# clayne/CPU-Raytracer

Measured on AMD Instinct MI355X. Metric: Mrays/s (primary+shadow+reflection+refraction), higher is better.
Workload: dtype f32

## Files before the change

### cpu-raytracer_amd/csrc/rtx_api.hip

```cpp
#include <hip/hip_runtime.h>
#include <stdio.h>
#include <stdlib.h>
#include <string.h>
#include <math.h>
#include <string>
#include <vector>
#include <algorithm>
#include <type_traits>

#include "../../include/rtx.h"
#include "rtx_device.h"
#include "rtx_math.h"
#include "rtx_libm.h"
#include "rtx_texture.h"
#include "rtx_trace.h"
#include "rtx_shade.h"
#include "rtx_packet.h"
#include "rtx_present.h"
#include "rtx_update.h"
#include "rtx_refit.h"
#include "rtx_build.h"
#include "rtx_normals.h"
#include "rtx_query.h"
#include "rtx_nearest.h"
// ... 153 lines not shown
    K.shade_grid = (int)knob_int("RTX_SHADE_GRID", 4, 1, 64);
    K.lane_from_level = (int)knob_int("RTX_LANE_FROM_LEVEL", -1, 0, 1 << 20);
    K.lane_from_level_any = (int)knob_int("RTX_LANE_FROM_LEVEL_ANY", -1, 0, 1 << 20);
    K.split_items = (int)knob_int("RTX_PK_SPLIT", 256, 0, 1 << 16);
    if (K.split_items > 0) K.split_items = (K.split_items + 63) & ~63;
    K.resolve_block = (int)knob_int("RTX_RESOLVE_BLOCK", 256, 64, 256);
    if (K.resolve_block != 64 && K.resolve_block != 128 && K.resolve_block != 256) K.resolve_block = 256;
    K.pk4_order = (int)knob_int("RTX_PK4_ORDER", 1, 0, 1);
    K.merge_any = knob_int("RTX_SERIAL_MERGE_ANY", 1, 0, 1) != 0;
    K.no_wide = knob_int("RTX_PK_WIDE", 1, 0, 1) == 0;
    K.lpt = (int)knob_int("RTX_PK_LPT", -1, -1, 1);
    K.graph = knob_int("RTX_GRAPH", 0, 0, 1) != 0;
    K.no_wide_closest = knob_int("RTX_PK_WIDE_CLOSEST", 1, 0, 1) == 0;
    K.fuse_shade = knob_int("RTX_FUSE_SHADE", 0, 0, 1) != 0;
    K.update_small_max = (int)knob_int("RTX_UPDATE_SMALL_MAX", RTX_UPDATE_SMALL_MAX, 0, RTX_UPDATE_SMALL_MAX);
    K.tex_pass_levels = (int)knob_int("RTX_TEX_PASS_LEVELS", rtxt::DEFAULT_PASS_LEVELS, 1, rtxt::MAX_PASS_LEVELS);
    c->nearest_fetch = knob_int("RTX_NEAREST_FETCH", 1, 0, 1) != 0;
    c->query_grid = (int)knob_int("RTX_QUERY_GRID", 0, 0, 1 << 20);
    K.fail_item_alloc = knob_int("RTX_DEBUG_FAIL_ITEM_ALLOC", 0, 0, 1) != 0;
    int bpc = 0;
    hipOccupancyMaxActiveBlocksPerMultiprocessor(&bpc, k_trace_fast<false>, RTX_TRACE_BLOCK, 0);
    c->trace_blocks_closest = c->n_cu * (bpc > 0 ? bpc : 2);
    hipOccupancyMaxActiveBlocksPerMultiprocessor(&bpc, k_trace_fast<true>, RTX_TRACE_BLOCK, 0);
    c->trace_blocks_any = c->n_cu * (bpc > 0 ? bpc : 2);
    hipOccupancyMaxActiveBlocksPerMultiprocessor(&bpc, k_trace<false, true>, RTX_TRACE_BLOCK, 0);
    c->trace_blocks_count = c->n_cu * (bpc > 0 ? bpc : 2);
    if (K.fuse_shade) hipOccupancyMaxActiveBlocksPerMultiprocessor(&bpc, k_packet<false, false, false, true, false>, RTX_PK_BLOCK, 0);
    else              hipOccupancyMaxActiveBlocksPerMultiprocessor(&bpc, k_packet<false, false>, RTX_PK_BLOCK, 0);
    c->pk_blocks_closest = (c->n_cu * (bpc > 0 ? bpc : 4) + 1) & ~1;
    hipOccupancyMaxActiveBlocksPerMultiprocessor(&bpc, k_packet<true, false>, RTX_PK_BLOCK, 0);
    c->pk_blocks_any = (c->n_cu * (bpc > 0 ? bpc : 4) + 1) & ~1;
    {
        const double f = knob_real("RTX_PK_GRID_SCALE", 1.0, 0.05, 16.0);
        if (f != 1.0) { c->pk_blocks_closest = ((int)(c->pk_blocks_closest * f) + 1) & ~1; c->pk_blocks_any = ((int)(c->pk_blocks_any * f) + 1) & ~1; }
        const double fa = knob_real("RTX_PK_GRID_ANY", 0.0, 0.05, 64.0), fc = knob_real("RTX_PK_GRID_CLOSEST", 0.0, 0.05, 64.0);
        if (fa > 0.0) c->pk_blocks_any = ((int)(c->n_cu * fa) + 1) & ~1;
        if (fc > 0.0) c->pk_blocks_closest = ((int)(c->n_cu * fc) + 1) & ~1;
    }
    {
        const int g = RTX_PK_CLASSES * RTX_WAVE / RTX_PK_BLOCK > 1 ? RTX_PK_CLASSES * RTX_WAVE / RTX_PK_BLOCK : 1;
        c->pk_blocks_any = (c->pk_blocks_any + g - 1) / g * g; c->pk_blocks_closest = (c->pk_blocks_closest + g - 1) / g * g;
        if (c->pk_blocks_any < g) c->pk_blocks_any = g;
        if (c->pk_blocks_closest < g) c->pk_blocks_closest = g;
    }
    long long max_threads = (long long)(c->trace_blocks_closest > c->trace_blocks_any ? c->trace_blocks_closest : c->trace_blocks_any) * RTX_TRACE_BLOCK;
    if ((long long)c->trace_blocks_count * RTX_TRACE_BLOCK > max_threads) max_threads = (long long)c->trace_blocks_count * RTX_TRACE_BLOCK;
    if ((long long)c->pk_blocks_any * RTX_PK_BLOCK > max_threads) max_threads = (long long)c->pk_blocks_any * RTX_PK_BLOCK;
    if ((long long)c->pk_blocks_closest * RTX_PK_BLOCK > max_threads) max_threads = (long long)c->pk_blocks_closest * RTX_PK_BLOCK;
    c->q.pk_defer_t0 = (int)knob_int("RTX_PK_DEFER", 8, 0, 64);
    c->q.pk_defer_leaf = (int)knob_int("RTX_PK_DEFER_LEAF", c->q.pk_defer_t0 / 2, 0, 64);
    c->q.pk_defer_t0_closest = (int)knob_int("RTX_PK_DEFER_CLOSEST", 64, 0, 64);
    c->q.pk_closest_asm = (int)knob_int("RTX_PK_CLOSEST_ASM", 1, 0, 1);
    c->q.pk_defer_t0_primary = (int)knob_int("RTX_PK_DEFER_PRIMARY", c->q.pk_closest_asm ? 4 : 64, 0, 64);
    c->q.pk_order = (int)knob_int("RTX_PK_ORDER", 1, 0, 1);
    c->q.prof_level = (int)knob_int("RTX_LANE_PROF_LEVEL", 2, 0, 100 + RTX_MAX_LEVELS);
    c->q.pk_defer_grow = (int)knob_int("RTX_PK_GROW", 3, 0, 31);
    c->q.spill_threads = (int)max_threads;
    rc = ensure(c, c->d_spill, (size_t)c->q.spill_threads * (RTX_MAX_STACK - RTX_LDS_STACK) * 4 * 3);
    if (!rc) rc = ensure(c, c->d_pk_fifo, (size_t)c->q.spill_threads * RTX_PK_FIFO * 8);
    { int ib = 0; hipOccupancyMaxActiveBlocksPerMultiprocessor(&ib, k_items, RTX_ITEM_BLOCK, 0); c->item_blocks = c->n_cu * (ib > 0 ? ib : 4);
      const double f = knob_real("RTX_ITEM_GRID", 0.0, 0.05, 64.0); if (f > 0.0) c->item_blocks = (int)(c->n_cu * f) > 0 ? (int)(c->n_cu * f) : 1; }
    c->q.pk_items = nullptr; c->q.pk_item_count = nullptr; c->q.pk_item_cap = 0;
    if (rc) { rtx_destroy(c); return rc; }
    *out_ctx = c;
    return RTX_OK;
}

extern "C" int rtx_destroy(rtx_ctx * c) {
    if (!c) return RTX_ERR_INVALID_ARG;
    hipSetDevice(c->cfg.device);
    if (c->stream) hipStreamSynchronize(c->stream);
    for (hipEvent_t e : c->event_pool) hipEventDestroy(e);
    if (c->graph_exec) { hipGraphExecDestroy(c->graph_exec); c->graph_exec = nullptr; }
    if (c->order_stream) { hipStreamSynchronize(c->order_stream); hipStreamDestroy(c->order_stream); hipEventDestroy(c->ev_cost); hipEventDestroy(c->ev_order); }
    if (c->any_stream) { hipStreamSynchronize(c->any_stream); hipStreamDestroy(c->any_stream); }
    if (c->ev_shade0) hipEventDestroy(c->ev_shade0);
    if (c->ev_shade_last) hipEventDestroy(c->ev_shade_last);
    if (c->ev_any_done) hipEventDestroy(c->ev_any_done);
    if (c->own_stream) hipStreamDestroy(c->own_stream);
    delete c;
    return RTX_OK;
}

static bool validate_tree(const rtx_bvh_node * nodes, int node_count, int64_t primitive_count, int * max_inner_depth = nullptr, int * max_leaf_count = nullptr) {
    if (node_count < 1) return false;
    std::vector<unsigned char> seen((size_t)node_count, 0);
    std::vector<std::pair<int, int>> stack(1, std::make_pair(0, 0));
    int deepest = -1, biggest = 0;
    while (!stack.empty()) {
        const int i = stack.back().first, d = stack.back().second; stack.pop_back();
        if (seen[i]) return false;
        seen[i] = 1;
        const int cnt = nodes[i].count & 0x3fffffff, f = nodes[i].left_or_first;
        if (cnt > 0) { if (f < 0 || (int64_t)f + cnt > primitive_count) return false; if (cnt > biggest) biggest = cnt; }
        else { if (f < 0 || f + 1 >= node_count) return false; if (d > deepest) deepest = d; stack.push_back(std::make_pair(f, d + 1)); stack.push_back(std::make_pair(f + 1, d + 1)); }
    }
    if (max_inner_depth) *max_inner_depth = deepest;
    if (max_leaf_count) *max_leaf_count = biggest;
    return true;
}


struct BlasStaged { DevBlas B; rtx_ctx::BlasHost H; };

template <typename T> static int stage_array(rtx_ctx * c, std::vector<DevBuf> & arrays, const void * src, size_t copy, size_t bytes, const T ** out) {
    DevBuf b;
// ... 2149 lines not shown
```

### cpu-raytracer_amd/csrc/rtx_packet.h

```cpp
#pragma once
#include "rtx_math.h"
#include "rtx_device.h"
#include "rtx_trace.h"
#include "rtx_shade.h"

#define RTX_PK_CLASSES  8
#ifndef RTX_PK_WAVES_ANY
#define RTX_PK_WAVES_ANY 5
#endif
#ifndef RTX_PK_WAVES_SPLIT
#define RTX_PK_WAVES_SPLIT 5
#endif
#ifndef RTX_PK_WAVES_CLOSEST
#define RTX_PK_WAVES_CLOSEST 4
#endif
#ifndef RTX_PK_CHUNK
#define RTX_PK_CHUNK 64u
#endif
#ifndef RTX_PK_WAVES_FUSED
#define RTX_PK_WAVES_FUSED 3
#endif

typedef const __attribute__((address_space(4))) rtx_f4v * rtx_cptr;
typedef float rtx_f2v __attribute__((ext_vector_type(2)));
RTX_D int rfl(int v) { return __builtin_amdgcn_readfirstlane(v); }
RTX_D unsigned long long rfl64(unsigned long long v) { return ((unsigned long long)(uint32_t)rfl((int)(uint32_t)(v >> 32)) << 32) | (unsigned long long)(uint32_t)rfl((int)(uint32_t)v); }
RTX_D rtx_cptr pk_cptr(const void * p) {
    const unsigned long long a = (unsigned long long)p;
    const unsigned long long u = ((unsigned long long)(uint32_t)rfl((int)(uint32_t)(a >> 32)) << 32) | (unsigned long long)(uint32_t)rfl((int)(uint32_t)a);
    return (rtx_cptr)u;
}
RTX_D float4 sld(rtx_cptr p, int i) { const rtx_f4v v = p[i]; return make_float4(v.x, v.y, v.z, v.w); }

RTX_D float pk_min(float a, float b) { float r; asm("v_min_f32 %0, %1, %2" : "=v"(r) : "v"(a), "v"(b)); return r; }
RTX_D float pk_max(float a, float b) { float r; asm("v_max_f32 %0, %1, %2" : "=v"(r) : "v"(a), "v"(b)); return r; }
RTX_D float pk_min3(float a, float b, float c) { float r; asm("v_min3_f32 %0, %1, %2, %3" : "=v"(r) : "v"(a), "v"(b), "v"(c)); return r; }
RTX_D float pk_max3(float a, float b, float c) { float r; asm("v_max3_f32 %0, %1, %2, %3" : "=v"(r) : "v"(a), "v"(b), "v"(c)); return r; }
RTX_D float pk_max_s(float s, float b) { float r; asm("v_max_f32 %0, %1, %2" : "=v"(r) : "s"(s), "v"(b)); return r; }

#define PK_FLAG_ITER      0x40000000
#define PK_FLAG_PRETESTED 0x20000000

enum { PKS_PACKETS, PKS_PAIR_STEPS, PKS_TRI_STEPS, PKS_PAIR_LANES, PKS_TRI_LANES };

struct PkRay {
    rtx_f2v o_xy, o_zz, i_xy, i_zz;
    v3 d;
    float tcur;
};
RTX_D void pk_set_ray(PkRay & r, v3 o, v3 d, v3 inv) {
    r.o_xy = rtx_f2v{ o.x, o.y }; r.o_zz = rtx_f2v{ o.z, o.z };
    r.i_xy = rtx_f2v{ inv.x, inv.y }; r.i_zz = rtx_f2v{ inv.z, inv.z };
    r.d = d;
}

template <bool FAST>
RTX_D bool pk_slab(float4 q0, float4 q1, const PkRay & r) {
    const rtx_f2v t0xy = (rtx_f2v{ q0.x, q0.y } - r.o_xy) * r.i_xy;
    const rtx_f2v t1xy = (rtx_f2v{ q0.z, q0.w } - r.o_xy) * r.i_xy;
    const rtx_f2v tz   = (rtx_f2v{ q1.x, q1.y } - r.o_zz) * r.i_zz;
    if (FAST) {
        const float t_near = pk_max_s(RAY_EPSILON, pk_max3(pk_min(t0xy.x, t1xy.x), pk_min(t0xy.y, t1xy.y), pk_min(tz.x, tz.y)));
        const float t_far  = pk_min(r.tcur, pk_min3(pk_max(t0xy.x, t1xy.x), pk_max(t0xy.y, t1xy.y), pk_max(tz.x, tz.y)));
        return t_near < t_far;
    }
    const float tminx = fmin_ref(t0xy.x, t1xy.x), tminy = fmin_ref(t0xy.y, t1xy.y), tminz = fmin_ref(tz.x, tz.y);
    const float tmaxx = fmax_ref(t0xy.x, t1xy.x), tmaxy = fmax_ref(t0xy.y, t1xy.y), tmaxz = fmax_ref(tz.x, tz.y);
    const float t_near = fmax_ref(fmax_ref(RAY_EPSILON, tminx), fmax_ref(tminy, tminz));
    const float t_far  = fmin_ref(fmin_ref(r.tcur, tmaxx), fmin_ref(tmaxy, tmaxz));
    return t_near < t_far;
}

struct Pk4Step { int e1, e2, e3; bool q1, q2, q3; bool have_cur; int cur_first, cur_cnt; };
RTX_D Pk4Step pk4_step(rtx_gptr nodes4, const int first, const PkRay & ray) {
    const int base = 4 * first;
    const float4 a0 = gld(nodes4, base), a1 = gld(nodes4, base + 1), b0 = gld(nodes4, base + 2), b1 = gld(nodes4, base + 3);
    const float4 c0 = gld(nodes4, base + 4), c1 = gld(nodes4, base + 5), d0 = gld(nodes4, base + 6), d1 = gld(nodes4, base + 7);
    const bool p0 = pk_slab<true>(a0, a1, ray), p1 = pk_slab<true>(b0, b1, ray), p2 = pk_slab<true>(c0, c1, ray), p3 = pk_slab<true>(d0, d1, ray);
    Pk4Step r;
    r.e1 = rtxl::wide_pack((uint32_t)as_i(b1.z), (uint32_t)as_i(b1.w)); r.q1 = p1 & p0;
    r.e2 = rtxl::wide_pack((uint32_t)as_i(c1.z), (uint32_t)as_i(c1.w)); r.q2 = p2 & (p0 | p1);
    r.e3 = rtxl::wide_pack((uint32_t)as_i(d1.z), (uint32_t)as_i(d1.w)); r.q3 = p3 & (p0 | p1 | p2);
    r.have_cur = p0 | p1 | p2 | p3;
    r.cur_first = p0 ? as_i(a1.z) : (p1 ? as_i(b1.z) : (p2 ? as_i(c1.z) : as_i(d1.z)));
    r.cur_cnt   = p0 ? as_i(a1.w) : (p1 ? as_i(b1.w) : (p2 ? as_i(c1.w) : as_i(d1.w)));
    return r;
}

#ifdef RTX_PK_PROF
#define PK_T0() const unsigned long long pk_t0_ = __builtin_amdgcn_s_memtime()
#define PK_T1(slot) do { W.prof[slot] += __builtin_amdgcn_s_memtime() - pk_t0_; W.prof[slot + 5]++; } while (0)
#else
#define PK_T0() do {} while (0)
#define PK_T1(slot) do {} while (0)
// ... 950 lines not shown
                fi++;
                if (fi < fifo_n) nxt = H.fifo[fi * H.fifo_stride];
                if (rtxl::ref_is_packed(e)) {
                    if (key < tcur) { cur_first = rtxl::ref_first(e); cur_cnt = rtxl::ref_count_word(e); have_cur = true; }
                } else {
                    const float4 na = gld(nodes, 2 * e), nb = gld(nodes, 2 * e + 1);
                    float k;
                    const bool pass = (key != key) ? slab_test_sel<true>(na, nb, co, cinv, tcur, k) : (key < tcur);
                    if (pass) { cur_first = as_i(na.w); cur_cnt = as_i(nb.w); have_cur = true; }
                }
            }
        }
#ifdef RTX_LANE_PROF
        { const unsigned long long lp_f = LP_NOW(); if (lp_popg || lp_fifo) W.lp[9] = (uint32_t)rfl((int)(W.lp[9] + (uint32_t)(lp_f - lp_d))); }
#endif
    }
#ifdef RTX_LANE_PROF
    {
        const unsigned long long lp_e = LP_NOW();
        W.lp[0] = (uint32_t)rfl((int)(W.lp[0] + (uint32_t)(lp_e - lp_t0))); W.lp[1] = (uint32_t)rfl((int)(W.lp[1] + (uint32_t)(lp_it))); W.lp[12] = (uint32_t)rfl((int)(W.lp[12] + 1u));
        if ((uint32_t)(lp_e - lp_t0) > W.lp[10]) W.lp[10] = (uint32_t)rfl((int)(uint32_t)(lp_e - lp_t0));
        if ((uint32_t)lp_it > W.lp[11]) W.lp[11] = (uint32_t)rfl((int)(uint32_t)lp_it);
    }
#endif
    W.ray.tcur = tcur;
    W.fifo_n = 0;
}

#define PK_ASM_REF  \
        "s_and_b32 s76, %[cnt], 0x3fffffff\n\t"                                                                                     \
        "s_cmp_lt_u32 s76, 16\n\t"                                                                                                  \
        "s_cselect_b32 s77, 1, 0\n\t"                                                                                               \
        "s_cmp_lt_u32 %[first], 0x1000000\n\t"                                                                                      \
        "s_cselect_b32 s78, 1, 0\n\t"                                                                                               \
        "s_and_b32 s77, s77, s78\n\t"                                                                                               \
        "s_lshr_b32 s78, %[cnt], 30\n\t"                                                                                            \
        "s_lshl_b32 s78, s78, 28\n\t"                                                                                               \
        "s_lshl_b32 s76, s76, 24\n\t"                                                                                               \
        "s_or_b32 s78, s78, s76\n\t"                                                                                                \
        "s_or_b32 s78, s78, %[first]\n\t"                                                                                           \
        "s_or_b32 s78, s78, 0x40000000\n\t"                                                                                         \
        "s_cmp_lg_u32 s77, 0\n\t"                                                                                                   \
        "s_cselect_b32 s79, s78, %[idx]\n\t"
#define PK_ASM_FIFO_APPEND(MASK_LO, MASK_HI, KEY)                         \
        "s_mov_b64 s[92:93], exec\n\t"                                                                                              \
        "s_mov_b32 exec_lo, " MASK_LO "\n\t"                                                                                        \
        "s_mov_b32 exec_hi, " MASK_HI "\n\t"                                                                                        \
        "v_mov_b32 v28, s79\n\t"                                                                                                    \
        "v_mov_b32 v29, " KEY "\n\t"                                                                                                \
        "global_store_dwordx2 %[fvoff], v[28:29], %[fbase]\n\t"                                                                     \
        "v_add_u32 %[fvoff], %[fstride], %[fvoff]\n\t"                                                                              \
        "v_add_u32 %[fn], 1, %[fn]\n\t"                                                                                             \
        "s_mov_b64 exec, s[92:93]\n\t"
RTX_D void pk_blas_closest_asm(PkWalk & W, const int stack_size, const int ordered, const PkHybrid & H, const int prim, const uint32_t gthread) {
    W.cur_first = rfl(W.cur_first); W.cur_cnt = rfl(W.cur_cnt); W.cur_idx = rfl(W.cur_idx); W.m = rfl64(W.m); W.sp = rfl(W.sp);
    W.depth = rfl(W.depth); W.pub = rfl64(W.pub);
    int err = 0, steps = rfl(W.pk_steps);
    const int floor_sp = rfl(W.floor_sp), ssz = rfl(stack_size), ord = rfl(ordered), t0d = rfl(H.t0), gsh = rfl(H.grow), primv = rfl(prim);
    const unsigned long long posx = __ballot(W.ray.d.x > 0.0f), posy = __ballot(W.ray.d.y > 0.0f), posz = __ballot(W.ray.d.z > 0.0f);
    const float eps = RAY_EPSILON;
    const unsigned long long nodes = rfl64((unsigned long long)W.nodes), tris = rfl64((unsigned long long)W.tris);
    const unsigned long long fbase = rfl64((unsigned long long)(H.fifo - gthread));
    const int fstride = rfl(H.fifo_stride * 8);
    uint32_t fvoff = (gthread + (uint32_t)W.fifo_n * (uint32_t)H.fifo_stride) * 8u;
    float t0, t1, t2, t3, t4, t5, t6, t7, t8, t9;
    asm volatile(
        "s_mov_b64 s[94:95], %[nodes]\n\t"
        "s_mov_b64 s[96:97], %[tris]\n\t"
        "s_cmp_eq_u64 %[m], 0\n\t"
        "s_cbranch_scc1 PKC_POP_%=\n\t"
        "PKC_DISPATCH_%=:\n\t"
        "s_bcnt1_i32_b64 s89, %[m]\n\t"
        "s_lshr_b32 s90, %[steps], %[gsh]\n\t"
        "s_add_i32 s90, s90, %[t0d]\n\t"
        "s_add_i32 %[steps], %[steps], 1\n\t"
        "s_cmp_le_u32 s89, s90\n\t"
        "s_cbranch_scc0 PKC_WALK_%=\n\t"
        "s_sub_i32 s90, %[sp], %[floor]\n\t"
        "s_add_i32 s90, s90, 2\n\t"
        "s_cmp_le_i32 s90, %[fifomax]\n\t"
        "s_cbranch_scc0 PKC_WALK_%=\n\t"
        "s_mov_b64 s[86:87], %[m]\n\t"
        PK_ASM_REF
        PK_ASM_FIFO_APPEND("s86", "s87", "0xff800000")
        "s_andn2_b64 %[pub], %[pub], %[m]\n\t"
        "s_branch PKC_POP_%=\n\t"
        "PKC_WALK_%=:\n\t"
        "s_and_b32 s88, %[cnt], 0x3fffffff\n\t"
        "s_cmp_lg_u32 s88, 0\n\t"
        "s_cbranch_scc1 PKC_LEAF_%=\n\t"
        "s_add_i32 s90, %[depth], 2\n\t"
        "s_cmp_gt_i32 s90, %[ssz]\n\t"
        "s_cselect_b32 %[err], 1, %[err]\n\t"
        "s_lshl_b32 s92, %[first], 5\n\t"
        "s_load_dwordx16 s[64:79], s[94:95], s92\n\t"
        "s_mov_b32 s91, 1\n\t"
        "s_cmp_eq_u32 %[ordered], 0\n\t"
        "s_cbranch_scc1 PKC_ORD_%=\n\t"
        "s_lshr_b32 s90, %[cnt], 30\n\t"
        "s_cmp_eq_u32 s90, 0\n\t"
        "s_cbranch_scc1 PKC_ORD_%=\n\t"
        "s_mov_b64 s[86:87], %[posx]\n\t"
        "s_cmp_eq_u32 s90, 2\n\t"
        "s_cselect_b64 s[86:87], %[posy], s[86:87]\n\t"
        "s_cmp_eq_u32 s90, 3\n\t"
        "s_cselect_b64 s[86:87], %[posz], s[86:87]\n\t"
        "s_and_b64 s[86:87], s[86:87], %[m]\n\t"
        "s_cmp_eq_u64 s[86:87], 0\n\t"
        "s_cselect_b32 s91, 0, 1\n\t"
        "s_cbranch_scc1 PKC_ORD_%=\n\t"
        "s_cmp_eq_u64 s[86:87], %[m]\n\t"
        "s_cbranch_scc1 PKC_ORD_%=\n\t"
        "s_andn2_b64 s[88:89], %[m], s[86:87]\n\t"
        "s_mov_b64 %[m], s[86:87]\n\t"
        "s_cmp_ge_i32 %[sp], 64\n\t"
        "s_cselect_b32 %[err], 1, %[err]\n\t"
        "s_cbranch_scc1 PKC_ORD_%=\n\t"
        "s_mov_b32 m0, %[sp]\n\t"
        "s_or_b32 s90, %[depth], 0x20000000\n\t"
        "v_writelane_b32 %[sta], %[first], m0\n\t"
        "v_writelane_b32 %[stb], %[cnt], m0\n\t"
        "v_writelane_b32 %[stmlo], s88, m0\n\t"
        "v_writelane_b32 %[stmhi], s89, m0\n\t"
        "v_writelane_b32 %[stdf], s90, m0\n\t"
        "v_writelane_b32 %[stidx], %[idx], m0\n\t"
        "s_add_i32 %[sp], %[sp], 1\n\t"
        "PKC_ORD_%=:\n\t"
        "s_waitcnt lgkmcnt(0)\n\t"
        PK_ASM_SLAB(64, 65, 66, 67, 68, 69, "s[82:83]")
        PK_ASM_SLAB(72, 73, 74, 75, 76, 77, "s[84:85]")
        "s_add_i32 s90, %[first], 1\n\t"
        "s_cmp_lg_u32 s91, 0\n\t"
        "s_cselect_b64 s[86:87], s[82:83], s[84:85]\n\t"
        "s_cselect_b64 s[88:89], s[84:85], s[82:83]\n\t"
        "s_cselect_b32 s80, s70, s78\n\t"
        "s_cselect_b32 s81, s71, s79\n\t"
        "s_cselect_b32 s92, s78, s70\n\t"
        "s_cselect_b32 s93, s79, s71\n\t"
        "s_cselect_b32 s82, %[first], s90\n\t"
        "s_cselect_b32 s83, s90, %[first]\n\t"
        "s_cmp_eq_u64 s[86:87], 0\n\t"
        "s_cbranch_scc1 PKC_NONEAR_%=\n\t"
        "s_cmp_eq_u64 s[88:89], 0\n\t"
        "s_cbranch_scc1 PKC_NOFAR_%=\n\t"
        "s_cmp_ge_i32 %[sp], 64\n\t"
        "s_cbranch_scc1 PKC_OVER_%=\n\t"
        "s_mov_b32 m0, %[sp]\n\t"
        "s_nop 0\n\t"
        "v_writelane_b32 %[sta], s92, m0\n\t"
        "v_writelane_b32 %[stb], s93, m0\n\t"
        "v_writelane_b32 %[stmlo], s88, m0\n\t"
        "v_writelane_b32 %[stmhi], s89, m0\n\t"
        "v_writelane_b32 %[stdf], %[depth], m0\n\t"
        "v_writelane_b32 %[stidx], s83, m0\n\t"
        "s_add_i32 %[sp], %[sp], 1\n\t"
        "PKC_NOFAR_%=:\n\t"
        "s_mov_b32 %[first], s80\n\t"
        "s_mov_b32 %[cnt], s81\n\t"
        "s_mov_b32 %[idx], s82\n\t"
        "s_mov_b64 %[m], s[86:87]\n\t"
        "s_add_i32 %[depth], %[depth], 1\n\t"
        "s_branch PKC_DISPATCH_%=\n\t"
        "PKC_OVER_%=:\n\t"
        "s_mov_b32 %[err], 1\n\t"
        "s_branch PKC_NOFAR_%=\n\t"
        "PKC_NONEAR_%=:\n\t"
        "s_cmp_eq_u64 s[88:89], 0\n\t"
        "s_cbranch_scc1 PKC_POP_%=\n\t"
        "s_mov_b32 %[first], s92\n\t"
        "s_mov_b32 %[cnt], s93\n\t"
        "s_mov_b32 %[idx], s83\n\t"
        "s_mov_b64 %[m], s[88:89]\n\t"
        "s_branch PKC_DISPATCH_%=\n\t"
        "PKC_LEAF_%=:\n\t"
        "s_mov_b32 s98, %[first]\n\t"
        "s_add_i32 s99, %[first], s88\n\t"
        "PKC_TRI_%=:\n\t"
        "s_lshl_b32 s89, s98, 6\n\t"
        "s_load_dwordx8 s[64:71], s[96:97], s89\n\t"
        "s_add_u32 s89, s89, 32\n\t"
        "s_load_dwordx4 s[72:75], s[96:97], s89\n\t"
        "s_waitcnt lgkmcnt(0)\n\t"
        "v_mul_f32 %[t0], s74, %[dy]\n\t"
        "v_mul_f32 %[t1], s73, %[dz]\n\t"
        "v_mul_f32 %[t2], s72, %[dz]\n\t"
        "v_mul_f32 %[t3], s74, %[dx]\n\t"
        "v_mul_f32 %[t4], s73, %[dx]\n\t"
        "v_mul_f32 %[t5], s72, %[dy]\n\t"
        "v_sub_f32 v24, %[t0], %[t1]\n\t"
        "v_sub_f32 v25, %[t2], %[t3]\n\t"
        "v_sub_f32 v26, %[t4], %[t5]\n\t"
        "v_mul_f32 %[t0], s69, v25\n\t"
        "v_mul_f32 %[t1], s70, v26\n\t"
        "v_mul_f32 %[t2], s68, v24\n\t"
        "v_add_f32 %[t0], %[t0], %[t1]\n\t"
        "v_add_f32 %[t9], %[t2], %[t0]\n\t"
        "v_div_scale_f32 %[t0], s[84:85], %[t9], %[t9], 1.0\n\t"
        "v_rcp_f32 %[t1], %[t0]\n\t"
        "v_div_scale_f32 %[t2], vcc, 1.0, %[t9], 1.0\n\t"
        "v_subrev_f32 v27, s64, %[ox]\n\t"
        "v_fma_f32 %[t3], -%[t0], %[t1], 1.0\n\t"
        "v_fmac_f32 %[t1], %[t3], %[t1]\n\t"
        "v_mul_f32 %[t4], %[t2], %[t1]\n\t"
        "v_fma_f32 %[t5], -%[t0], %[t4], %[t2]\n\t"
        "v_fmac_f32 %[t4], %[t5], %[t1]\n\t"
        "v_fma_f32 %[t0], -%[t0], %[t4], %[t2]\n\t"
// ... 35 lines not shown
        "v_add_f32 %[t0], %[t2], %[t0]\n\t"
        "v_mul_f32 %[t5], %[t8], %[t0]\n\t"
        "v_add_f32 %[t4], %[t7], %[t6]\n\t"
        "v_cmp_lt_f32 s[86:87], 0, %[t6]\n\t"
        "s_and_b64 s[84:85], s[84:85], s[86:87]\n\t"
        "v_cmp_gt_f32 s[86:87], 1.0, %[t4]\n\t"
        "s_and_b64 s[84:85], s[84:85], s[86:87]\n\t"
        "v_cmp_lt_f32 s[86:87], %[eps], %[t5]\n\t"
        "s_and_b64 s[84:85], s[84:85], s[86:87]\n\t"
        "v_cmp_lt_f32 s[86:87], %[t5], %[tcur]\n\t"
        "s_and_b64 s[84:85], s[84:85], s[86:87]\n\t"
        "s_cmp_lg_u64 s[84:85], 0\n\t"
        "s_cbranch_scc0 PKC_NEXT_%=\n\t"
        "s_mov_b64 s[92:93], exec\n\t"
        "s_mov_b64 exec, s[84:85]\n\t"
        "v_mov_b32 %[tcur], %[t5]\n\t"
        "v_mov_b32 %[bu], %[t7]\n\t"
        "v_mov_b32 %[bv], %[t6]\n\t"
        "v_mov_b32 %[btri], s98\n\t"
        "v_mov_b32 %[bprim], %[prim]\n\t"
        "s_mov_b64 exec, s[92:93]\n\t"
        "PKC_NEXT_%=:\n\t"
        "s_add_i32 s98, s98, 1\n\t"
        "s_cmp_lt_i32 s98, s99\n\t"
        "s_cbranch_scc1 PKC_TRI_%=\n\t"
        "PKC_POP_%=:\n\t"
        "s_mov_b64 %[m], 0\n\t"
        "s_cmp_le_i32 %[sp], %[floor]\n\t"
        "s_cbranch_scc1 PKC_END_%=\n\t"
        "s_sub_i32 %[sp], %[sp], 1\n\t"
        "s_mov_b32 m0, %[sp]\n\t"
        "s_nop 0\n\t"
        "v_readlane_b32 s84, %[stmlo], m0\n\t"
        "v_readlane_b32 s85, %[stmhi], m0\n\t"
        "v_readlane_b32 %[first], %[sta], m0\n\t"
        "v_readlane_b32 %[cnt], %[stb], m0\n\t"
        "v_readlane_b32 s91, %[stdf], m0\n\t"
        "v_readlane_b32 %[idx], %[stidx], m0\n\t"
        "s_and_b32 %[depth], s91, 0xffff\n\t"
        "s_bitcmp1_b32 s91, 29\n\t"
        "s_cbranch_scc0 PKC_FAR_%=\n\t"
        "s_andn2_b64 s[86:87], s[84:85], %[pub]\n\t"
        "s_cmp_lg_u64 s[86:87], 0\n\t"
        "s_cbranch_scc0 PKC_PRE_PUB_%=\n\t"
        PK_ASM_REF
        PK_ASM_FIFO_APPEND("s86", "s87", "0xff800000")
        "PKC_PRE_PUB_%=:\n\t"
        "s_and_b64 %[m], s[84:85], %[pub]\n\t"
        "s_cmp_eq_u64 %[m], 0\n\t"
        "s_cbranch_scc1 PKC_POP_%=\n\t"
        "s_branch PKC_DISPATCH_%=\n\t"
        "PKC_FAR_%=:\n\t"
        "s_mov_b64 %[m], s[84:85]\n\t"
        "s_lshl_b32 s88, %[idx], 5\n\t"
        "s_load_dwordx8 s[64:71], s[94:95], s88\n\t"
        "s_waitcnt lgkmcnt(0)\n\t"
        PK_ASM_SLAB(64, 65, 66, 67, 68, 69, "s[80:81]")
        "s_andn2_b64 s[86:87], s[80:81], %[pub]\n\t"
        "s_cmp_lg_u64 s[86:87], 0\n\t"
        "s_cbranch_scc0 PKC_FAR_PUB_%=\n\t"
        PK_ASM_REF
        PK_ASM_FIFO_APPEND("s86", "s87", "v30")
        "PKC_FAR_PUB_%=:\n\t"
        "s_and_b64 %[m], s[80:81], %[pub]\n\t"
        "s_cmp_eq_u64 %[m], 0\n\t"
        "s_cbranch_scc1 PKC_POP_%=\n\t"
        "s_branch PKC_DISPATCH_%=\n\t"
        "PKC_END_%=:\n\t"
        : [first] "+&s"(W.cur_first), [cnt] "+&s"(W.cur_cnt), [idx] "+&s"(W.cur_idx), [m] "+&s"(W.m), [sp] "+&s"(W.sp), [depth] "+&s"(W.depth),
          [err] "+&s"(err), [steps] "+&s"(steps), [pub] "+&s"(W.pub),
          [sta] "+&v"(W.st_a), [stb] "+&v"(W.st_b), [stmlo] "+&v"(W.st_mlo), [stmhi] "+&v"(W.st_mhi), [stdf] "+&v"(W.st_df), [stidx] "+&v"(W.st_idx),
          [tcur] "+&v"(W.ray.tcur), [bu] "+&v"(W.best_u), [bv] "+&v"(W.best_v), [btri] "+&v"(W.best_tri), [bprim] "+&v"(W.best_prim),
          [fvoff] "+&v"(fvoff), [fn] "+&v"(W.fifo_n),
          [t0] "=&v"(t0), [t1] "=&v"(t1), [t2] "=&v"(t2), [t3] "=&v"(t3), [t4] "=&v"(t4), [t5] "=&v"(t5), [t6] "=&v"(t6), [t7] "=&v"(t7),
          [t8] "=&v"(t8), [t9] "=&v"(t9)
        : [nodes] "s"(nodes), [tris] "s"(tris), [floor] "s"(floor_sp), [ssz] "s"(ssz), [eps] "s"(eps), [ordered] "s"(ord), [t0d] "s"(t0d), [gsh] "s"(gsh),
          [posx] "s"(posx), [posy] "s"(posy), [posz] "s"(posz), [fbase] "s"(fbase), [fstride] "s"(fstride), [prim] "s"(primv), [fifomax] "s"((int)RTX_PK_FIFO),
          [oxy] "v"(W.ray.o_xy), [ozz] "v"(W.ray.o_zz), [ixy] "v"(W.ray.i_xy), [izz] "v"(W.ray.i_zz),
          [ox] "v"(W.ray.o_xy.x), [oy] "v"(W.ray.o_xy.y), [oz] "v"(W.ray.o_zz.x), [dx] "v"(W.ray.d.x), [dy] "v"(W.ray.d.y), [dz] "v"(W.ray.d.z)
        : "vcc", "scc", "m0", "memory",
          "s64", "s65", "s66", "s67", "s68", "s69", "s70", "s71", "s72", "s73", "s74", "s75", "s76", "s77", "s78", "s79",
          "s80", "s81", "s82", "s83", "s84", "s85", "s86", "s87", "s88", "s89", "s90", "s91", "s92", "s93", "s94", "s95", "s96", "s97", "s98", "s99",
          "v24", "v25", "v26", "v27", "v28", "v29", "v30", "v31");
    W.pk_steps = steps;
    if (err) W.err = 1;
}

template <bool ANY, bool PSTAT, bool FAST, bool ASM, bool SPLIT, typename WorldFn>
RTX_D bool pk_walk(const DevScene & sc, PkWalk & W, const int lane, const bool ordered, const PkHybrid & H, WorldFn && world) {
    for (;;) {
        if (W.m != 0ull) {
            if (!ANY && ASM && FAST && W.floor_sp >= 0) {
                const int thr = H.t0 + (W.pk_steps >> H.grow);
                if (__popcll(W.m) <= thr && (W.sp - W.floor_sp) + 2 <= RTX_PK_FIFO) {
                    if ((W.m >> lane) & 1ull) { H.fifo[W.fifo_n * H.fifo_stride] = make_int2(W.cur_idx, as_i(PK_KEY_PASSED)); W.fifo_n++; }
                    W.pub &= ~W.m; W.m = 0ull;
                    continue;
                }
                W.pk_steps++;
            }
            const int leafc = W.cur_cnt & 0x3fffffff;
            if (leafc > 0) {
                PK_T0();
                if (W.floor_sp >= 0) {
                    const v3 co = V3(W.ray.o_xy.x, W.ray.o_xy.y, W.ray.o_zz.x), cd = W.ray.d;
                    for (int i = W.cur_first; i < W.cur_first + leafc; i++) {
                        const float4 p0 = sld(W.tris, RTX_TRI_STRIDE * i), e1 = sld(W.tris, RTX_TRI_STRIDE * i + 1), e2 = sld(W.tris, RTX_TRI_STRIDE * i + 2);
                        if (PSTAT) { W.st_tris++; W.st_tri_lanes += (unsigned long long)__popcll(W.m); }
                        float t, u, v;
                        const bool hit = tri_test_all(v3q(p0), v3q(e1), v3q(e2), co, cd, W.ray.tcur, t, u, v);
                        const unsigned long long hm = __ballot(hit) & W.m;
                        if (hm != 0ull) {
                            const bool mine = (hm >> lane) & 1ull;
                            if (ANY) { if (mine) W.occluded = true; W.alive &= ~hm; W.m &= ~hm; if (W.m == 0ull) break; }
                            else if (mine) { W.ray.tcur = t; W.best_u = u; W.best_v = v; W.best_tri = i; W.best_prim = PRIM_TRI | W.cur_inst; }
                        }
                    }
                } else {
                    pk_push<ANY>(W, W.cur_first, leafc, W.m, 0, PK_FLAG_ITER);
                }
                W.m = 0ull;
                PK_T1(2);
            } else if (ASM && FAST) {
                PK_T0();
                pk_descend<ANY>(W, sc.stack_size, ordered ? 1 : 0, (!ANY && W.floor_sp >= 0) ? H.t0 + (W.pk_steps >> H.grow) : -1);
                PK_T1(1);
            } else {
                if (W.depth + 2 > sc.stack_size) W.err = 1;
                int left_first = 1;
                if (ordered) {
// ... 21 lines not shown
                if (m_near != 0ull) {
                    if (m_far != 0ull) pk_push<ANY>(W, far_first, far_cnt, m_far, far_idx, W.depth);
                    W.cur_idx = rfl(near_idx); W.cur_first = rfl(near_first); W.cur_cnt = rfl(near_cnt); W.m = m_near; W.depth = rfl(W.depth + 1);
                } else if (m_far != 0ull) {
                    W.cur_idx = rfl(far_idx); W.cur_first = rfl(far_first); W.cur_cnt = rfl(far_cnt); W.m = m_far;
                } else W.m = 0ull;
            }
            continue;
        }
        PK_T0();
        if (ANY && W.alive == 0ull) return true;
        if (W.floor_sp >= 0 && W.sp == W.floor_sp) {
            if (!ANY && ASM && FAST && W.pub != W.alive) {
                if (W.lane_nodes4c) pk_lane_phase_closest<true>(W, lane, ordered, H, W.lane_nodes, W.lane_nodes4c, W.lane_tris);
                else pk_lane_phase_closest<false>(W, lane, ordered, H, W.lane_nodes, nullptr, W.lane_tris);
                W.pub = W.alive;
            }
            if (W.sp == 0) return true;
            W.floor_sp = -1; W.nodes = W.tlas;
            v3 o, d; world(o, d);
            pk_set_ray(W.ray, o, d, vrcp(d));
        }
        if (W.sp == 0) return true;
        W.sp--;
        const int ea = __builtin_amdgcn_readlane(W.st_a, W.sp), eb = __builtin_amdgcn_readlane(W.st_b, W.sp);
        const int edf = __builtin_amdgcn_readlane(W.st_df, W.sp);
        const unsigned long long em = ((unsigned long long)(uint32_t)__builtin_amdgcn_readlane(W.st_mhi, W.sp) << 32) |
                                      (unsigned long long)(uint32_t)__builtin_amdgcn_readlane(W.st_mlo, W.sp);
        unsigned long long pm = em & W.alive;
        if (!ANY && ASM && FAST && (pm & ~W.pub) != 0ull) {
            if (((pm & ~W.pub) >> lane) & 1ull) {
                H.fifo[W.fifo_n * H.fifo_stride] = make_int2(__builtin_amdgcn_readlane(W.st_idx, W.sp), (edf & PK_FLAG_PRETESTED) ? as_i(PK_KEY_PASSED) : 0x7fc00000); W.fifo_n++;
            }
            pm &= W.pub;
        }
        if (pm == 0ull) continue;
        if (edf & PK_FLAG_ITER) {
            if (eb > 1) pk_push<ANY>(W, ea + 1, eb - 1, pm, 0, PK_FLAG_ITER);
            const int inst = rfl(sc.tlas_indices[ea]);
            const rtx_instance & I = sc.instances[inst];
            v3 o, d; world(o, d);
            const v3 co = xform_pos(I.world_inv, o), cd = xform_dir(I.world_inv, d), cinv = vrcp(cd);
            pk_set_ray(W.ray, co, cd, cinv);
            W.cur_blas = rfl(I.blas_id);
            const DevBlas & B = sc.blas[W.cur_blas];
            W.nodes = pk_cptr(B.pk_nodes); W.tris = pk_cptr(B.tri_hot); W.cur_inst = inst;
            W.lane_nodes = RTX_GPTR(B.nodes); W.lane_tris = RTX_GPTR(B.tri_hot); if (!ANY) W.lane_nodes4c = RTX_GPTR(B.pk4c_nodes);
            W.floor_sp = W.sp; W.depth = 0;
            const float4 na = sld(W.nodes, 0), nb = sld(W.nodes, 1);
            const bool risky = FAST && __ballot(W.valid && !inv_is_finite(cinv) && pk_nan_possible(B, co, cinv)) != 0ull;
            W.m = (risky ? __ballot(pk_slab<false>(na, nb, W.ray)) : __ballot(pk_slab<FAST>(na, nb, W.ray))) & pm;
            W.cur_idx = 0; W.cur_first = as_i(nb.z); W.cur_cnt = as_i(nb.w);
            if (risky) return false;
            if (ASM && FAST && !ANY && H.closest_asm) {
#ifdef RTX_LANE_PROF
                asm volatile("s_waitcnt vmcnt(0) lgkmcnt(0)" ::: "memory"); const unsigned long long sw_t0 = __builtin_amdgcn_s_memtime(); const int sw_s0 = W.pk_steps;
#endif
#ifdef RTX_PK_SKIPWALK
                W.m = 0ull;
#else
                pk_blas_closest_asm(W, sc.stack_size, ordered ? 1 : 0, H, PRIM_TRI | inst, H.gthread);
#endif
#ifdef RTX_LANE_PROF
                asm volatile("s_waitcnt vmcnt(0) lgkmcnt(0)" ::: "memory");
                W.lp[13] = (uint32_t)rfl((int)(W.lp[13] + (uint32_t)(__builtin_amdgcn_s_memtime() - sw_t0))); W.lp[14] = (uint32_t)rfl((int)(W.lp[14] + (uint32_t)(W.pk_steps - sw_s0)));
                W.lp[15] = (uint32_t)rfl((int)(W.lp[15] + 1u));
#endif
            }
            if (ASM && FAST && ANY) {
                PK_T0();
                W.psp = 0;
                if (SPLIT) {
#ifdef RTX_PK_SKIPWALK
                    W.m = 0ull;
#else
                    pk_blas_any_asm4(W, pk_cptr(B.pk4_nodes), H.lane_lds, H.t0, H.t_leaf, H.grow, H.item_cap, H.item_base, W.item_slot);
#endif
                    PK_T1(1);
                } else if (B.pk4_nodes) {
                    pk_blas_any_asm4(W, pk_cptr(B.pk4_nodes), H.lane_lds, H.t0, H.t_leaf, H.grow, 0u, 0ull, 0u);
                    PK_T1(1);
                    if (W.alive != 0ull && __ballot(W.psp > 0) != 0ull) { PK_T0(); pk_lane_phase_any4(W, lane, H.lane_lds, H.spill, H.spill_stride, RTX_GPTR(B.pk4_nodes), RTX_GPTR(B.tri_hot)); PK_T1(2); }
                } else {
                    pk_blas_any_asm(W, sc.stack_size, H.lane_lds, H.t0, H.grow);
                    PK_T1(1);
                    if (W.alive != 0ull && __ballot(W.psp > 0) != 0ull) { PK_T0(); pk_lane_phase_any(W, lane, H.stk, H.spill, H.spill_stride, RTX_GPTR(B.nodes), RTX_GPTR(B.tri_hot)); PK_T1(2); }
                }
            }
        } else {
            W.m = pm;
            if (!ANY && !(edf & PK_FLAG_PRETESTED)) {
                const int eidx = __builtin_amdgcn_readlane(W.st_idx, W.sp);
                const float4 na = sld(W.nodes, 2 * eidx), nb = sld(W.nodes, 2 * eidx + 1);
                W.m = __ballot(pk_slab<FAST>(na, nb, W.ray)) & pm;
                W.cur_idx = eidx;
            } else if (!ANY) W.cur_idx = __builtin_amdgcn_readlane(W.st_idx, W.sp);
            W.cur_first = rfl(ea); W.cur_cnt = rfl(eb); W.depth = rfl(edf & 0xffff);
        }
        PK_T1(3);
    }
}

template <bool ANY, bool PSTAT, bool SPLIT = false, bool FUSE = false, bool CULL = false, int VIEWS = 0>
__global__ __launch_bounds__(RTX_PK_BLOCK, ANY ? (SPLIT ? RTX_PK_WAVES_SPLIT : RTX_PK_WAVES_ANY) : (FUSE ? RTX_PK_WAVES_FUSED : RTX_PK_WAVES_CLOSEST))
void k_packet(const DevScene sc, const DevQueues q, const int level, const int level_hi) {
    __shared__ int s_priv[RTX_PK_BLOCK / RTX_WAVE][SPLIT ? 1 : (ANY ? RTX_PK_PRIV : 2 * RTX_LDS_STACK)][RTX_WAVE];
    const int lane = threadIdx.x & 63;
    PkHybrid H;
    H.stk = &s_priv[threadIdx.x >> 6][0][lane];
    H.stk_key = (float *)&s_priv[threadIdx.x >> 6][(ANY || SPLIT) ? 0 : RTX_LDS_STACK][lane];
    H.lane_lds = (uint32_t)(uintptr_t)H.stk;
    H.spill_stride = q.spill_threads;
    {
        const size_t region = (size_t)q.spill_threads * (RTX_MAX_STACK - RTX_LDS_STACK), gt = blockIdx.x * blockDim.x + threadIdx.x;
// ... 307 lines not shown
```

Measured before the change: 9595.

## Specialize closest-hit packet slab tests for direction-coherent packets and cache far-child keys

```diff
diff --git a/cpu-raytracer_amd/csrc/rtx_api.hip b/cpu-raytracer_amd/csrc/rtx_api.hip
--- a/cpu-raytracer_amd/csrc/rtx_api.hip
+++ b/cpu-raytracer_amd/csrc/rtx_api.hip
@@ -229,6 +229,7 @@
     c->q.pk_defer_t0_closest = (int)knob_int("RTX_PK_DEFER_CLOSEST", 64, 0, 64);
     c->q.pk_closest_asm = (int)knob_int("RTX_PK_CLOSEST_ASM", 1, 0, 1);
     c->q.pk_defer_t0_primary = (int)knob_int("RTX_PK_DEFER_PRIMARY", c->q.pk_closest_asm ? 4 : 64, 0, 64);
+    c->q.pk_closest_asm |= (int)knob_int("RTX_PK_COHERENT", 15, 0, 15) << PK_COH_SHIFT;
     c->q.pk_order = (int)knob_int("RTX_PK_ORDER", 1, 0, 1);
     c->q.prof_level = (int)knob_int("RTX_LANE_PROF_LEVEL", 2, 0, 100 + RTX_MAX_LEVELS);
     c->q.pk_defer_grow = (int)knob_int("RTX_PK_GROW", 3, 0, 31);
diff --git a/cpu-raytracer_amd/csrc/rtx_packet.h b/cpu-raytracer_amd/csrc/rtx_packet.h
--- a/cpu-raytracer_amd/csrc/rtx_packet.h
+++ b/cpu-raytracer_amd/csrc/rtx_packet.h
@@ -40,6 +40,12 @@
 
 #define PK_FLAG_ITER      0x40000000
 #define PK_FLAG_PRETESTED 0x20000000
+#define PK_FLAG_NOKEY     0x10000000
+#define PK_COH_SHIFT      8
+#define PK_COH_SIGN       1
+#define PK_COH_KEYS       4
+#define PK_COH_ORDER      8
+#define PK_COH_ALL        (PK_COH_SIGN | PK_COH_KEYS | PK_COH_ORDER)
 
 enum { PKS_PACKETS, PKS_PAIR_STEPS, PKS_TRI_STEPS, PKS_PAIR_LANES, PKS_TRI_LANES };
 
@@ -1096,12 +1102,65 @@
         "v_add_u32 %[fvoff], %[fstride], %[fvoff]\n\t"                                                                              \
         "v_add_u32 %[fn], 1, %[fn]\n\t"                                                                                             \
         "s_mov_b64 exec, s[92:93]\n\t"
-RTX_D void pk_blas_closest_asm(PkWalk & W, const int stack_size, const int ordered, const PkHybrid & H, const int prim, const uint32_t gthread) {
+#define PKC_ASM_SLAB(X0, X1, X2, X3, X4, X5, MASK, TN)                                                                              \
+    "v_pk_add_f32 v[24:25], s[" #X0 ":" #X1 "], %[oxy] neg_lo:[0,1] neg_hi:[0,1]\n\t"                                              \
+    "v_pk_add_f32 v[26:27], s[" #X2 ":" #X3 "], %[oxy] neg_lo:[0,1] neg_hi:[0,1]\n\t"                                              \
+    "v_pk_add_f32 v[28:29], s[" #X4 ":" #X5 "], %[ozz] neg_lo:[0,1] neg_hi:[0,1]\n\t"                                              \
+    "v_pk_mul_f32 v[24:25], %[ixy], v[24:25]\n\t"                                                                                   \
+    "v_pk_mul_f32 v[26:27], %[ixy], v[26:27]\n\t"                                                                                   \
+    "v_pk_mul_f32 v[28:29], %[izz], v[28:29]\n\t"                                                                                   \
+    "v_min_f32 " TN ", v24, v26\n\t"                                                                                                \
+    "v_max_f32 v24, v24, v26\n\t"                                                                                                   \
+    "v_min_f32 v31, v25, v27\n\t"                                                                                                   \
+    "v_max_f32 v25, v25, v27\n\t"                                                                                                   \
+    "v_min_f32 v26, v28, v29\n\t"                                                                                                   \
+    "v_max_f32 v27, v28, v29\n\t"                                                                                                   \
+    "v_max3_f32 " TN ", " TN ", v31, v26\n\t"                                                                                       \
+    "v_min3_f32 v24, v24, v25, v27\n\t"                                                                                             \
+    "v_max_f32 " TN ", %[eps], " TN "\n\t"                                                                                          \
+    "v_min_f32 v24, %[tcur], v24\n\t"                                                                                               \
+    "v_cmp_lt_f32 vcc, " TN ", v24\n\t"                                                                                             \
+    "s_and_b64 " MASK ", vcc, %[m]\n\t"
+#define PKC_ASM_SLAB_S(X0, X1, X2, X3, X4, X5, MASK, TN, NX, FX, NY, FY, NZ, FZ)                                                     \
+    "v_pk_add_f32 v[24:25], s[" #X0 ":" #X1 "], %[oxy] neg_lo:[0,1] neg_hi:[0,1]\n\t"                                              \
+    "v_pk_add_f32 v[26:27], s[" #X2 ":" #X3 "], %[oxy] neg_lo:[0,1] neg_hi:[0,1]\n\t"                                              \
+    "v_pk_add_f32 v[28:29], s[" #X4 ":" #X5 "], %[ozz] neg_lo:[0,1] neg_hi:[0,1]\n\t"                                              \
+    "v_pk_mul_f32 v[24:25], %[ixy], v[24:25]\n\t"                                                                                   \
+    "v_pk_mul_f32 v[26:27], %[ixy], v[26:27]\n\t"                                                                                   \
+    "v_pk_mul_f32 v[28:29], %[izz], v[28:29]\n\t"                                                                                   \
+    "v_max3_f32 " TN ", " NX ", " NY ", " NZ "\n\t"                                                                                 \
+    "v_min3_f32 v31, " FX ", " FY ", " FZ "\n\t"                                                                                    \
+    "v_max_f32 " TN ", %[eps], " TN "\n\t"                                                                                          \
+    "v_min_f32 v31, %[tcur], v31\n\t"                                                                                               \
+    "v_cmp_lt_f32 vcc, " TN ", v31\n\t"                                                                                             \
+    "s_and_b64 " MASK ", vcc, %[m]\n\t"
+#define PKC_ASM_PAIR_S(NX, FX, NY, FY, NZ, FZ)                                                                                      \
+    PKC_ASM_SLAB_S(64, 65, 66, 67, 68, 69, "s[82:83]", "%[t0]", NX, FX, NY, FY, NZ, FZ)                                             \
+    PKC_ASM_SLAB_S(72, 73, 74, 75, 76, 77, "s[84:85]", "v30", NX, FX, NY, FY, NZ, FZ)                                               \
+    "s_branch PKC_SEL_%=\n\t"
+#define PKC_ASM_ONE_S(NX, FX, NY, FY, NZ, FZ)                                                                                       \
+    PKC_ASM_SLAB_S(64, 65, 66, 67, 68, 69, "s[80:81]", "v30", NX, FX, NY, FY, NZ, FZ)                                               \
+    "s_branch PKC_FAR_TESTED_%=\n\t"
+RTX_D void pk_blas_closest_asm(PkWalk & W, const int stack_size, const int ordered, const PkHybrid & H, const int prim, const uint32_t gthread, const int coh) {
     W.cur_first = rfl(W.cur_first); W.cur_cnt = rfl(W.cur_cnt); W.cur_idx = rfl(W.cur_idx); W.m = rfl64(W.m); W.sp = rfl(W.sp);
     W.depth = rfl(W.depth); W.pub = rfl64(W.pub);
     int err = 0, steps = rfl(W.pk_steps);
-    const int floor_sp = rfl(W.floor_sp), ssz = rfl(stack_size), ord = rfl(ordered), t0d = rfl(H.t0), gsh = rfl(H.grow), primv = rfl(prim);
+    const int floor_sp = rfl(W.floor_sp), ssz = rfl(stack_size), t0d = rfl(H.t0), gsh = rfl(H.grow), primv = rfl(prim);
+    int ord; asm("v_readfirstlane_b32 %0, %1" : "=s"(ord) : "v"(ordered));
     const unsigned long long posx = __ballot(W.ray.d.x > 0.0f), posy = __ballot(W.ray.d.y > 0.0f), posz = __ballot(W.ray.d.z > 0.0f);
+    int cf = 8;
+    if (coh & PK_COH_SIGN) {
+        const unsigned long long nx = __ballot(W.ray.i_xy.x < 0.0f) & W.m, ny = __ballot(W.ray.i_xy.y < 0.0f) & W.m, nz = __ballot(W.ray.i_zz.x < 0.0f) & W.m;
+        if (!((nx != 0ull && nx != W.m) || (ny != 0ull && ny != W.m) || (nz != 0ull && nz != W.m))) cf = (nx != 0ull ? 1 : 0) | (ny != 0ull ? 2 : 0) | (nz != 0ull ? 4 : 0);
+    }
+    if (coh & PK_COH_ORDER) {
+        const unsigned long long px = posx & W.m, py = posy & W.m, pz = posz & W.m;
+        if (!((px != 0ull && px != W.m) || (py != 0ull && py != W.m) || (pz != 0ull && pz != W.m))) cf |= 0x110 | (px != 0ull ? 0x200 : 0) | (py != 0ull ? 0x400 : 0) | (pz != 0ull ? 0x800 : 0);
+    }
+    cf = rfl(cf);
+    const int krows = rfl((coh & PK_COH_KEYS) ? 2 * RTX_LDS_STACK : 0);
+    const uint32_t llds = H.lane_lds;
+    unsigned long long jt = 0ull;
     const float eps = RAY_EPSILON;
     const unsigned long long nodes = rfl64((unsigned long long)W.nodes), tris = rfl64((unsigned long long)W.tris);
     const unsigned long long fbase = rfl64((unsigned long long)(H.fifo - gthread));
@@ -1111,6 +1170,14 @@
     asm volatile(
         "s_mov_b64 s[94:95], %[nodes]\n\t"
         "s_mov_b64 s[96:97], %[tris]\n\t"
+        "s_getpc_b64 s[92:93]\n\t"
+        "PKC_PC_%=:\n\t"
+        "s_and_b32 s90, %[cf], 15\n\t"
+        "s_mul_i32 s90, s90, PKC_V1_%=-PKC_V0_%=\n\t"
+        "s_add_u32 s90, s90, PKC_V0_%=-PKC_PC_%=\n\t"
+        "s_add_u32 s92, s92, s90\n\t"
+        "s_addc_u32 s93, s93, 0\n\t"
+        "s_mov_b64 %[jt], s[92:93]\n\t"
         "s_cmp_eq_u64 %[m], 0\n\t"
         "s_cbranch_scc1 PKC_POP_%=\n\t"
         "PKC_DISPATCH_%=:\n\t"
@@ -1138,6 +1205,14 @@
         "s_cselect_b32 %[err], 1, %[err]\n\t"
         "s_lshl_b32 s92, %[first], 5\n\t"
         "s_load_dwordx16 s[64:79], s[94:95], s92\n\t"
+        "s_bitcmp1_b32 %[cf], 4\n\t"
+        "s_cbranch_scc0 PKC_ORDG_%=\n\t"
+        "s_lshr_b32 s90, %[cnt], 30\n\t"
+        "s_add_i32 s90, s90, 8\n\t"
+        "s_bitcmp1_b32 %[cf], s90\n\t"
+        "s_cselect_b32 s91, 1, 0\n\t"
+        "s_branch PKC_ORD_%=\n\t"
+        "PKC_ORDG_%=:\n\t"
         "s_mov_b32 s91, 1\n\t"
         "s_cmp_eq_u32 %[ordered], 0\n\t"
         "s_cbranch_scc1 PKC_ORD_%=\n\t"
@@ -1171,8 +1246,20 @@
         "s_add_i32 %[sp], %[sp], 1\n\t"
         "PKC_ORD_%=:\n\t"
         "s_waitcnt lgkmcnt(0)\n\t"
-        PK_ASM_SLAB(64, 65, 66, 67, 68, 69, "s[82:83]")
-        PK_ASM_SLAB(72, 73, 74, 75, 76, 77, "s[84:85]")
+        "s_setpc_b64 %[jt]\n\t"
+        "PKC_V0_%=:\n\t"
+        PKC_ASM_PAIR_S("v24", "v26", "v25", "v27", "v28", "v29")
+        "PKC_V1_%=:\n\t"
+        PKC_ASM_PAIR_S("v26", "v24", "v25", "v27", "v28", "v29")
+        PKC_ASM_PAIR_S("v24", "v26", "v27", "v25", "v28", "v29")
+        PKC_ASM_PAIR_S("v26", "v24", "v27", "v25", "v28", "v29")
+        PKC_ASM_PAIR_S("v24", "v26", "v25", "v27", "v29", "v28")
+        PKC_ASM_PAIR_S("v26", "v24", "v25", "v27", "v29", "v28")
+        PKC_ASM_PAIR_S("v24", "v26", "v27", "v25", "v29", "v28")
+        PKC_ASM_PAIR_S("v26", "v24", "v27", "v25", "v29", "v28")
+        PKC_ASM_SLAB(64, 65, 66, 67, 68, 69, "s[82:83]", "%[t0]")
+        PKC_ASM_SLAB(72, 73, 74, 75, 76, 77, "s[84:85]", "v30")
+        "PKC_SEL_%=:\n\t"
         "s_add_i32 s90, %[first], 1\n\t"
         "s_cmp_lg_u32 s91, 0\n\t"
         "s_cselect_b64 s[86:87], s[82:83], s[84:85]\n\t"
@@ -1190,12 +1277,24 @@
         "s_cmp_ge_i32 %[sp], 64\n\t"
         "s_cbranch_scc1 PKC_OVER_%=\n\t"
         "s_mov_b32 m0, %[sp]\n\t"
-        "s_nop 0\n\t"
+        "s_sub_i32 s90, %[sp], %[floor]\n\t"
+        "s_cmp_lt_u32 s90, %[krows]\n\t"
+        "s_cbranch_scc0 PKC_NOKEY_%=\n\t"
+        "s_cmp_lg_u32 s91, 0\n\t"
+        "s_cselect_b64 vcc, -1, 0\n\t"
+        "v_cndmask_b32 %[t1], %[t0], v30, vcc\n\t"
+        "v_lshl_add_u32 %[t2], s90, 8, %[llds]\n\t"
+        "ds_write_b32 %[t2], %[t1]\n\t"
+        "v_writelane_b32 %[stdf], %[depth], m0\n\t"
+        "s_branch PKC_PUSH_%=\n\t"
+        "PKC_NOKEY_%=:\n\t"
+        "s_or_b32 s90, %[depth], 0x10000000\n\t"
+        "v_writelane_b32 %[stdf], s90, m0\n\t"
+        "PKC_PUSH_%=:\n\t"
         "v_writelane_b32 %[sta], s92, m0\n\t"
         "v_writelane_b32 %[stb], s93, m0\n\t"
         "v_writelane_b32 %[stmlo], s88, m0\n\t"
         "v_writelane_b32 %[stmhi], s89, m0\n\t"
-        "v_writelane_b32 %[stdf], %[depth], m0\n\t"
         "v_writelane_b32 %[stidx], s83, m0\n\t"
         "s_add_i32 %[sp], %[sp], 1\n\t"
         "PKC_NOFAR_%=:\n\t"
@@ -1337,10 +1436,53 @@
         "s_branch PKC_DISPATCH_%=\n\t"
         "PKC_FAR_%=:\n\t"
         "s_mov_b64 %[m], s[84:85]\n\t"
+        "s_bitcmp1_b32 s91, 28\n\t"
+        "s_cbranch_scc1 PKC_FAR_BOX_%=\n\t"
+        "s_sub_i32 s88, %[sp], %[floor]\n\t"
+        "v_lshl_add_u32 %[t2], s88, 8, %[llds]\n\t"
+        "ds_read_b32 v30, %[t2]\n\t"
+        "s_waitcnt lgkmcnt(0)\n\t"
+        "v_cmp_lt_f32 vcc, v30, %[tcur]\n\t"
+        "s_and_b64 s[80:81], vcc, %[m]\n\t"
+        "s_branch PKC_FAR_TESTED_%=\n\t"
+        "PKC_FAR_BOX_%=:\n\t"
         "s_lshl_b32 s88, %[idx], 5\n\t"
         "s_load_dwordx8 s[64:71], s[94:95], s88\n\t"
         "s_waitcnt lgkmcnt(0)\n\t"
-        PK_ASM_SLAB(64, 65, 66, 67, 68, 69, "s[80:81]")
+        "s_bitcmp1_b32 %[cf], 3\n\t"
+        "s_cbranch_scc1 PKC_F8_%=\n\t"
+        "s_bitcmp1_b32 %[cf], 2\n\t"
+        "s_cbranch_scc1 PKC_F4_%=\n\t"
+        "s_bitcmp1_b32 %[cf], 1\n\t"
+        "s_cbranch_scc1 PKC_F2_%=\n\t"
+        "s_bitcmp1_b32 %[cf], 0\n\t"
+        "s_cbranch_scc1 PKC_F1_%=\n\t"
+        PKC_ASM_ONE_S("v24", "v26", "v25", "v27", "v28", "v29")
+        "PKC_F1_%=:\n\t"
+        PKC_ASM_ONE_S("v26", "v24", "v25", "v27", "v28", "v29")
+        "PKC_F2_%=:\n\t"
+        "s_bitcmp1_b32 %[cf], 0\n\t"
+        "s_cbranch_scc1 PKC_F3_%=\n\t"
+        PKC_ASM_ONE_S("v24", "v26", "v27", "v25", "v28", "v29")
+        "PKC_F3_%=:\n\t"
+        PKC_ASM_ONE_S("v26", "v24", "v27", "v25", "v28", "v29")
+        "PKC_F4_%=:\n\t"
+        "s_bitcmp1_b32 %[cf], 1\n\t"
+        "s_cbranch_scc1 PKC_F6_%=\n\t"
+        "s_bitcmp1_b32 %[cf], 0\n\t"
+        "s_cbranch_scc1 PKC_F5_%=\n\t"
+        PKC_ASM_ONE_S("v24", "v26", "v25", "v27", "v29", "v28")
+        "PKC_F5_%=:\n\t"
+        PKC_ASM_ONE_S("v26", "v24", "v25", "v27", "v29", "v28")
+        "PKC_F6_%=:\n\t"
+        "s_bitcmp1_b32 %[cf], 0\n\t"
+        "s_cbranch_scc1 PKC_F7_%=\n\t"
+        PKC_ASM_ONE_S("v24", "v26", "v27", "v25", "v29", "v28")
+        "PKC_F7_%=:\n\t"
+        PKC_ASM_ONE_S("v26", "v24", "v27", "v25", "v29", "v28")
+        "PKC_F8_%=:\n\t"
+        PKC_ASM_SLAB(64, 65, 66, 67, 68, 69, "s[80:81]", "v30")
+        "PKC_FAR_TESTED_%=:\n\t"
         "s_andn2_b64 s[86:87], s[80:81], %[pub]\n\t"
         "s_cmp_lg_u64 s[86:87], 0\n\t"
         "s_cbranch_scc0 PKC_FAR_PUB_%=\n\t"
@@ -1356,11 +1498,12 @@
           [err] "+&s"(err), [steps] "+&s"(steps), [pub] "+&s"(W.pub),
           [sta] "+&v"(W.st_a), [stb] "+&v"(W.st_b), [stmlo] "+&v"(W.st_mlo), [stmhi] "+&v"(W.st_mhi), [stdf] "+&v"(W.st_df), [stidx] "+&v"(W.st_idx),
           [tcur] "+&v"(W.ray.tcur), [bu] "+&v"(W.best_u), [bv] "+&v"(W.best_v), [btri] "+&v"(W.best_tri), [bprim] "+&v"(W.best_prim),
-          [fvoff] "+&v"(fvoff), [fn] "+&v"(W.fifo_n),
+          [fvoff] "+&v"(fvoff), [fn] "+&v"(W.fifo_n), [jt] "+&s"(jt),
           [t0] "=&v"(t0), [t1] "=&v"(t1), [t2] "=&v"(t2), [t3] "=&v"(t3), [t4] "=&v"(t4), [t5] "=&v"(t5), [t6] "=&v"(t6), [t7] "=&v"(t7),
           [t8] "=&v"(t8), [t9] "=&v"(t9)
         : [nodes] "s"(nodes), [tris] "s"(tris), [floor] "s"(floor_sp), [ssz] "s"(ssz), [eps] "s"(eps), [ordered] "s"(ord), [t0d] "s"(t0d), [gsh] "s"(gsh),
           [posx] "s"(posx), [posy] "s"(posy), [posz] "s"(posz), [fbase] "s"(fbase), [fstride] "s"(fstride), [prim] "s"(primv), [fifomax] "s"((int)RTX_PK_FIFO),
+          [cf] "s"(cf), [krows] "s"(krows), [llds] "v"(llds),
           [oxy] "v"(W.ray.o_xy), [ozz] "v"(W.ray.o_zz), [ixy] "v"(W.ray.i_xy), [izz] "v"(W.ray.i_zz),
           [ox] "v"(W.ray.o_xy.x), [oy] "v"(W.ray.o_xy.y), [oz] "v"(W.ray.o_zz.x), [dx] "v"(W.ray.d.x), [dy] "v"(W.ray.d.y), [dz] "v"(W.ray.d.z)
         : "vcc", "scc", "m0", "memory",
@@ -1488,14 +1631,15 @@
             W.m = (risky ? __ballot(pk_slab<false>(na, nb, W.ray)) : __ballot(pk_slab<FAST>(na, nb, W.ray))) & pm;
             W.cur_idx = 0; W.cur_first = as_i(nb.z); W.cur_cnt = as_i(nb.w);
             if (risky) return false;
-            if (ASM && FAST && !ANY && H.closest_asm) {
+            if (ASM && FAST && !ANY && (H.closest_asm & 1)) {
 #ifdef RTX_LANE_PROF
                 asm volatile("s_waitcnt vmcnt(0) lgkmcnt(0)" ::: "memory"); const unsigned long long sw_t0 = __builtin_amdgcn_s_memtime(); const int sw_s0 = W.pk_steps;
 #endif
 #ifdef RTX_PK_SKIPWALK
                 W.m = 0ull;
 #else
-                pk_blas_closest_asm(W, sc.stack_size, ordered ? 1 : 0, H, PRIM_TRI | inst, H.gthread);
+                pk_blas_closest_asm(W, sc.stack_size, ordered ? 1 : 0, H, PRIM_TRI | inst, H.gthread,
+                                    (H.closest_asm >> PK_COH_SHIFT) & (B.pk4_nodes ? PK_COH_ALL : (PK_COH_ALL & ~PK_COH_SIGN)));
 #endif
 #ifdef RTX_LANE_PROF
                 asm volatile("s_waitcnt vmcnt(0) lgkmcnt(0)" ::: "memory");
```

Result: no change. 9685 (median of 6 runs) (+0.9%).
